# JanEGerken/HEAL-SWIN

Measured on AMD Instinct MI355X. Metric: images/sec fwd+bwd, HEAL-SWIN nside=256 seg, batch=8 at 1/2/4/8 MI355X, higher is better.
Workload: dtype bf16

## Files before the change

### heal_swin_amd/_lib.py

```python
import ctypes
import os

import numpy as np

_PKG = os.path.dirname(os.path.abspath(__file__))
LIB_PATH = os.path.join(_PKG, "lib", "libhealswin.so")

HS_F32, HS_BF16 = 0, 1
HS_F64 = 3
HS_PRED_LABELS, HS_PRED_ROWS16 = 2, 4
HS_ATTN_COSINE = 1
HS_ATTN_FORCE_VALU = 2
HS_ATTN_RESIDUAL = 4
HS_ATTN_OVERWRITE_GRADS = 8
HS_EPI_BIAS, HS_EPI_GELU, HS_EPI_DGELU, HS_EPI_RESID = 0, 1, 2, 3
HS_ACC_DEFER = 2
HS_MLP_NORM_AFTER = 16
HS_U8, HS_I32, HS_I64 = 8, 9, 10
HS_FLAT_PATCH_ROWS, HS_FLAT_PIXEL_ROWS, HS_FLAT_IMAGE = 0, 1, 2
HS_DEPTH_L1, HS_DEPTH_L2, HS_DEPTH_HUBER, HS_DEPTH_LOGVAR = 0, 1, 2, 3
HS_DT_NONE, HS_DT_LOG, HS_DT_INV = 0, 1, 2
HS_DT_ZERO_BKG, HS_DT_1000_BKG, HS_DT_AFFINE, HS_DT_INVERSE = 1, 2, 4, 8
HS_DEPTH_STATS_WORDS = 15

c_i64 = ctypes.c_int64
c_int = ctypes.c_int
c_uint = ctypes.c_uint
c_ptr = ctypes.c_void_p
c_float = ctypes.c_float


class WgradProblem(ctypes.Structure):
    _fields_ = [("dy", c_ptr), ("x", c_ptr), ("dw", c_ptr), ("dbias", c_ptr), ("n_out", c_int), ("k_in", c_int), ("accumulate", c_int),
                ("gelu_x", c_int)]


def wgrad_problems(members):
    arr = (WgradProblem * len(members))()
# ... 339 lines not shown
```

### heal_swin_amd/csrc/gemm_nt.hip

```cpp
#include <cstdlib>

#include "hs_gelu.h"

namespace hs {
HS_DEFINE_SEED_EPOCH_SETTER(set_seed_epoch_gemm_nt)

#ifdef HS_GEMM_TRACE
#define HS_GEMM_TRACE_PARAM uint64_t* trace;
constexpr int kTraceCap = 240;
static uint64_t* g_trace = nullptr;
extern "C" int hs_gemm_nt_set_trace(void* buf) {
    g_trace = (uint64_t*)buf;
    return 0;
}
template <typename Params>
void trace_attach(Params& p) {
    p.trace = g_trace;
}
constexpr int trace_lds(int used, int nw) { return used + nw * kTraceCap * 8 <= 163840 ? nw * kTraceCap * 8 : 0; }
struct Trace {
    uint64_t* out;
    bool on;
    int n = 0, nw, wave, lane;
    uint32_t base;
// ... 21 lines not shown
        }
    }
};
#else
#define HS_GEMM_TRACE_PARAM
template <typename Params>
void trace_attach(Params&) {}
constexpr int trace_lds(int, int) { return 0; }
struct Trace {
    template <typename Params>
    __device__ __forceinline__ Trace(const Params&, bool, uint32_t, int, int, int) {}
    __device__ __forceinline__ void operator()(int) const {}
    __device__ __forceinline__ void flush() const {}
};
#endif

namespace {

typedef unsigned int u32x2 __attribute__((__vector_size__(8)));
typedef unsigned int u32x4v __attribute__((__vector_size__(16)));

constexpr int kStoreAux = 2;
constexpr int kInAux = 2;
enum { EPI_BIAS = 0, EPI_GELU = 1, EPI_DGELU = 2, EPI_RESID = 3 };
constexpr int64_t kMaxRecords = 0x7FFFFE00;

struct GemmParams {
    const uint16_t *a, *b;
    int64_t lda, ldb;
    int k;
    const uint16_t *a2, *b2;
    int64_t lda2, ldb2;
    int k2;
    const float* bias;
    uint16_t* c;
    uint16_t* aux;
    int64_t m;
    int n;
    int tiles_n, tiles, per_xcd, blocks_per_xcd;
    float drop_p;
    uint64_t seed;
    HS_GEMM_TRACE_PARAM
};

template <int BM_, int BN_, int WM_, int WN_, int NSTAGE_, bool ALIAS_, int WGS_PER_CU_>
struct TileTraits {
    static constexpr int BM = BM_, BN = BN_, WM = WM_, WN = WN_, NSTAGE = NSTAGE_, WGS_PER_CU = WGS_PER_CU_;
    static constexpr bool ALIAS = ALIAS_;
    static constexpr int NW = WM * WN;
    static constexpr int TM = BM / WM / 32, TN = BN / WN / 32;
    static constexpr int AB = BM * 128, BB = BN * 128, STAGE = AB + BB;
    static constexpr int AHEAD = NSTAGE - 1;
    static_assert(TN == 2 && (TM == 2 || TM == 4), "the kernel is written for wave tiles of 64 columns and 64 or 128 rows");
    static_assert(!ALIAS || NW * 4096 <= STAGE, "patches do not fit a stage buffer");
    static_assert(BN * 4 <= 1024, "a bias slot holds one 1-KB DMA piece");

    static constexpr bool has_in(int epi) { return epi == EPI_DGELU || epi == EPI_RESID; }
    static constexpr bool ring(int epi) { return has_in(epi) && ALIAS && TM == 4 && STAGE >= NW * 8192; }
    static constexpr bool lbias(int epi) { return ALIAS && epi != EPI_DGELU; }
    static constexpr int NSLOT = NSTAGE + 1;
    static constexpr int PATCH_OFF = NSTAGE * STAGE;
    static constexpr int BIAS_OFF = NSTAGE * STAGE + (ALIAS ? 0 : NW * 4096);
    static constexpr int bias_lds(int epi) { return lbias(epi) ? NSLOT * 1024 : 0; }
    static constexpr int trace_off(int epi) { return BIAS_OFF + bias_lds(epi); }
    static constexpr int lds_bytes(int epi) { return trace_off(epi) + trace_lds(trace_off(epi), NW); }
};
using Tile1 = TileTraits<128, 128, 2, 2, 2, false, 2>;
using Tile2 = TileTraits<256, 128, 4, 2, 3, true, 1>;
using Tile3 = TileTraits<256, 256, 2, 4, 2, true, 1>;

constexpr int epi_younger_ops(int tm, int i) {
    const int stores = i < 2 ? i : 1;
    const int last_d = i + 1 < tm - 1 ? i + 1 : tm - 1;
    return 4 * (stores + (last_d - i));
}

template <int OFF>
__device__ __forceinline__ u32x4 lds_read_b128(uint32_t addr) {
    u32x4 v;
    asm volatile("ds_read_b128 %0, %1 offset:%2" : "=v"(v) : "v"(addr), "n"(OFF));
    return v;
}
// ... 31 lines not shown
        for (int j = 0; j < J; ++j) off[j] = row[j] * ((int)ld * 2) + col[j];
        ld32 = (int)ld * 64;
    }
    __device__ __forceinline__ void issue(unsigned char* stage, int wave, int q, int kb, int kseg) const {
        lds_void* dst = (lds_void*)(stage + LDS + (wave * N + q) * 1024);
        if constexpr (SC) {
            __builtin_amdgcn_raw_ptr_buffer_load_lds(rsrc, dst, 16, (uint32_t)off[q % J], kb + (q >> 2) * ld32, 0, 0);
        } else {
            const uint32_t voff = kb + col[q] < kseg ? (uint32_t)(off[q] + kb) : kOob;
            __builtin_amdgcn_raw_ptr_buffer_load_lds(rsrc, dst, 16, voff, 0, 0, 0);
        }
    }
};
__device__ __forceinline__ uint32_t frag_addr(uint32_t lds_base, int r, int half) {
    const int R = r >> 1;
    return lds_base + R * 256 + (((((r & 1) << 3) + half) ^ (R & 15)) << 4);
}

template <typename Tile, int EPI, bool DROP, bool FAST>
__global__ void __launch_bounds__(Tile::NW * 64, 2) gemm_nt_kernel(GemmParams p) {
#if defined(__HIP_DEVICE_COMPILE__)
    constexpr int BM = Tile::BM, BN = Tile::BN, WM = Tile::WM, WN = Tile::WN, NW = Tile::NW, TM = Tile::TM, TN = Tile::TN;
    constexpr int NSTAGE = Tile::NSTAGE, AHEAD = Tile::AHEAD, NSLOT = Tile::NSLOT, STAGE = Tile::STAGE, BIAS_OFF = Tile::BIAS_OFF;
    constexpr bool ALIAS = Tile::ALIAS, HAS_IN = Tile::has_in(EPI), RING = Tile::ring(EPI), LBIAS = Tile::lbias(EPI);
    constexpr int IW = FAST ? NW / 2 : NW;
    using OperandA = Operand<Tile::AB / 1024 / IW, 0, FAST>;
    using OperandB = Operand<Tile::BB / 1024 / IW, Tile::AB, FAST>;
    constexpr int PIECES = OperandA::N + OperandB::N;
    static_assert(Tile::lds_bytes(EPI) <= 163840, "LDS of one workgroup exceeds 160 KB");
    __shared__ __attribute__((aligned(16))) unsigned char smem[Tile::lds_bytes(EPI)];

    const int tid = threadIdx.x, lane = tid & 63, half = lane >> 5, l31 = lane & 31;
    const int wave = __builtin_amdgcn_readfirstlane(tid >> 6);
    const int wm = wave / WN, wn = wave % WN;

    const int xcd = blockIdx.x & 7, lb = blockIdx.x >> 3;
    const int id_end = min((xcd + 1) * p.per_xcd, p.tiles);
    const int id0 = xcd * p.per_xcd + lb;
    if (id0 >= id_end) return;
    const int nk1 = (p.k + 63) >> 6, nk2 = (p.k2 + 63) >> 6, nk = nk1 + nk2;
    struct Origin {
        int64_t m0;
        int n0;
    };
    auto tile_origin = [&](int id) {
        const int tm = id / p.tiles_n, tn = id - tm * p.tiles_n;
// ... 88 lines not shown
            constexpr int rest = PIECES - ks * PQ, cnt = rest < 0 ? 0 : rest < PQ ? rest : PQ;
            wait_frags(ks_c, Int<(ks < 3 ? TM + TN : 0)>{});
            mma(ks_c, Int<ks * PQ>{}, Int<cnt>{});
            if constexpr (ks + 2 < 4) read_frags(Int<ks + 2>{});
        });
    };

    const uint32_t own_rel = wave * 4096 + l31 * 128 + 8 * half;
    const uint32_t own_out_rel = wave * 4096 + l31 * 128 + 8 * (half ^ ((l31 >> 3) & 1));
    const uint32_t row_rel = wave * 4096 + (lane >> 3) * 128 + (((lane & 7) ^ (lane >> 3)) << 4);
    const bool second_half = ((half ^ (lane & (p.n >> 2))) & 1) != 0;
    auto epilogue = [&](int id, int buf_done, int slot_c) {
        const uint32_t patch_off = ALIAS ? buf_done * STAGE : Tile::PATCH_OFF;
        TR(10);
        if (ALIAS) __builtin_amdgcn_s_barrier();
        TR(11);
        const Origin o = tile_origin(id);
        const int64_t m0 = o.m0;
        const int n2 = p.n * 2;
        const int64_t cbytes = (p.m - m0) * (int64_t)n2;
        const __amdgpu_buffer_rsrc_t rc = clamped_rsrc(p.c + m0 * p.n, p.c ? cbytes : 0);
        const __amdgpu_buffer_rsrc_t rx = clamped_rsrc(p.aux + m0 * p.n, p.aux ? cbytes : 0);
        const ElemRng rng(p.drop_p, p.seed);
        const bool wide = RING || (p.n & 7) == 0;
        const int ncol0 = o.n0 + wn * (BN / WN);
        auto col_of = [&](int j, int g) { return ncol0 + j * 32 + 4 * half + 8 * g; };
        float4 bias4[TN][4];
        const uint32_t baddr = lds0 + BIAS_OFF + slot_c * 1024 + (wn * (BN / WN) + 4 * half) * 4;
        auto lds_bias = [&](int j, float4 (&b)[4]) {
            u32x4 bq[4];
#pragma unroll
            for (int g = 0; g < 4; ++g) asm volatile("ds_read_b128 %0, %1" : "=v"(bq[g]) : "v"(baddr + (j * 32 + 8 * g) * 4));
            asm volatile("s_waitcnt lgkmcnt(0)" : "+v"(bq[0]), "+v"(bq[1]), "+v"(bq[2]), "+v"(bq[3]));
#pragma unroll
            for (int g = 0; g < 4; ++g) b[g] = __builtin_bit_cast(float4, bq[g]);
        };
        if constexpr (!LBIAS) {
#pragma unroll
            for (int j = 0; j < TN; ++j)
#pragma unroll
                for (int g = 0; g < 4; ++g) {
                    const int n = col_of(j, g);
                    bias4[j][g] = (EPI != EPI_DGELU && p.bias && n < p.n) ? *(const float4*)(p.bias + n) : make_float4(0.f, 0.f, 0.f, 0.f);
                }
        }
        const int rl_col = ncol0 + (lane & 7) * 8;
        const uint32_t rl_voff = rl_col < p.n ? (uint32_t)((lane >> 3) * n2 + rl_col * 2) : kOob;
        auto row_soff = [&](int i, int t) -> int { return (wm * (BM / WM) + i * 32 + 8 * t) * n2; };
        const int in_col = ncol0 + (((lane & 7) ^ (lane >> 3)) << 3);
        const uint32_t in_voff = in_col < p.n ? (uint32_t)((lane >> 3) * n2 + in_col * 2) : kOob;
        auto request_in = [&](int i) {
            unsigned char* base = smem + patch_off + (i & 1) * (NW * 4096) + wave * 4096;
#pragma unroll
            for (int t = 0; t < 4; ++t)
                __builtin_amdgcn_raw_ptr_buffer_load_lds(rx, (lds_void*)(base + t * 1024), 16, in_voff, row_soff(i, t), 0, kInAux);
        };
        if constexpr (RING) {
            request_in(0);
            request_in(1);
        }
#pragma unroll
        for (int i = 0; i < TM; ++i) {
            const int ml = wm * (BM / WM) + i * 32 + l31;
            auto direct_off = [&](int j, int g) { return col_of(j, g) < p.n ? (uint32_t)(ml * n2 + col_of(j, g) * 2) : kOob; };
            const uint32_t pbase = lds0 + patch_off + (RING ? (i & 1) * (NW * 4096) : 0);
            const uint32_t own_addr = pbase + own_rel, row_addr = pbase + row_rel, own_out = pbase + own_out_rel;
// ... 25 lines not shown
                } else {
#pragma unroll
                    for (int j = 0; j < TN; ++j)
#pragma unroll
                        for (int g = 0; g < 4; ++g) xin[j][g] = __builtin_amdgcn_raw_buffer_load_b64(rx, direct_off(j, g), 0, 0);
                }
            }
            auto chunk_key = [&](int j, int g) { return rng.chunk_key((uint64_t)((m0 + ml) * p.n + col_of(j, g)) >> 3); };
            auto keep2 = [&](uint32_t ck, int t) {
                const uint32_t hh = ElemRng::pair_bits(ck, ElemRng::half_mult(second_half, t));
                return f32x2{rng.keep_lo(hh), rng.keep_hi(hh)};
            };
            u32x2 o1[TN][4], o2[TN][4];
#pragma unroll
            for (int j = 0; j < TN; ++j) {
                if constexpr (LBIAS) lds_bias(j, bias4[j]);
#pragma unroll
                for (int g = 0; g < 4; ++g) {
                    f32x16& a16 = acc[j][i];
                    f32x2 v[2] = {f32x2{a16[4 * g], a16[4 * g + 1]} + f32x2{bias4[j][g].x, bias4[j][g].y},
                                  f32x2{a16[4 * g + 2], a16[4 * g + 3]} + f32x2{bias4[j][g].z, bias4[j][g].w}};
                    uint32_t ck = 0;
                    if (DROP) ck = chunk_key(j, g);
                    if (EPI == EPI_GELU) {
                        o1[j][g] = pack_bf16x4(v[0], v[1]);
                        a16[4 * g] = v[0].x; a16[4 * g + 1] = v[0].y; a16[4 * g + 2] = v[1].x; a16[4 * g + 3] = v[1].y;
                        continue;
                    } else {
                        if (EPI == EPI_DGELU || EPI == EPI_RESID) {
#pragma unroll
                            for (int t = 0; t < 2; ++t) {
                                const f32x2 x = {__uint_as_float(xin[j][g][t] << 16), __uint_as_float(xin[j][g][t] & 0xffff0000u)};
                                if (EPI == EPI_DGELU) {
                                    v[t] *= gelu_grad2(x);
                                    if (DROP) v[t] *= keep2(ck, t);
                                } else {
                                    v[t] += x;
                                }
                            }
                        }
                        o1[j][g] = pack_bf16x4(v[0], v[1]);
                    }
#pragma unroll
                    for (int r = 0; r < 4; ++r) a16[4 * g + r] = 0.f;
                }
            }
            auto make_o2 = [&]() {
#pragma unroll
                for (int j = 0; j < TN; ++j)
#pragma unroll
                    for (int g0 = 0; g0 < 4; g0 += 2) {
                        f32x16& a16 = acc[j][i];
                        f32x2 v[4] = {f32x2{a16[4 * g0], a16[4 * g0 + 1]}, f32x2{a16[4 * g0 + 2], a16[4 * g0 + 3]},
                                      f32x2{a16[4 * g0 + 4], a16[4 * g0 + 5]}, f32x2{a16[4 * g0 + 6], a16[4 * g0 + 7]}};
#pragma unroll
                        for (int t = 0; t < 4; ++t) v[t] = gelu2(v[t]);
#pragma unroll
                        for (int gg = 0; gg < 2; ++gg) {
                            const int g = g0 + gg;
                            if (DROP) {
                                const uint32_t ck = chunk_key(j, g);
#pragma unroll
                                for (int t = 0; t < 2; ++t) v[2 * gg + t] *= keep2(ck, t);
                            }
                            o2[j][g] = pack_bf16x4(v[2 * gg], v[2 * gg + 1]);
#pragma unroll
                            for (int r = 0; r < 4; ++r) a16[4 * g + r] = 0.f;
                        }
                    }
            };
            TR(20);
            auto emit = [&](const __amdgpu_buffer_rsrc_t& rs, const u32x2 (&o)[TN][4]) {
                if (wide) {
#pragma unroll
                    for (int j = 0; j < TN; ++j)
#pragma unroll
                        for (int g = 0; g < 4; ++g)
                            asm volatile("ds_write_b64 %0, %1" ::"v"(own_out + (((4 * j + g) ^ (l31 & 7)) << 4)), "v"(o[j][g]) : "memory");
                    u32x4 rws[4];
                    asm volatile("ds_read_b128 %0, %1" : "=v"(rws[0]) : "v"(row_addr));
                    asm volatile("ds_read2_b64 %0, %1 offset0:129 offset1:128" : "=v"(rws[1]) : "v"(row_addr));
                    asm volatile("ds_read_b128 %0, %1 offset:2048" : "=v"(rws[2]) : "v"(row_addr));
                    asm volatile("ds_read2_b64 %0, %1 offset0:129 offset1:128" : "=v"(rws[3]) : "v"(row_addr + 2048));
                    asm volatile("s_waitcnt lgkmcnt(0)" : "+v"(rws[0]), "+v"(rws[1]), "+v"(rws[2]), "+v"(rws[3]));
                    TR(22);
#pragma unroll
                    for (int t = 0; t < 4; ++t)
                        __builtin_amdgcn_raw_buffer_store_b128(__builtin_bit_cast(u32x4v, rws[t]), rs, rl_voff, row_soff(i, t), kStoreAux);
                    asm volatile("s_nop 0" ::"v"(rws[0]), "v"(rws[1]), "v"(rws[2]), "v"(rws[3]));
                } else {
#pragma unroll
                    for (int j = 0; j < TN; ++j)
#pragma unroll
                        for (int g = 0; g < 4; ++g) __builtin_amdgcn_raw_buffer_store_b64(o[j][g], rs, direct_off(j, g), 0, kStoreAux);
                }
            };
            if (EPI == EPI_GELU) {
                if (NW == 8 && wave >= NW / 2) {
                    make_o2();
                    emit(rx, o2);
                    TR(21);
                    __builtin_amdgcn_sched_barrier(0);
                    if (p.c) emit(rc, o1);
                } else {
                    if (p.c) emit(rc, o1);
                    TR(21);
                    __builtin_amdgcn_sched_barrier(0);
                    make_o2();
                    emit(rx, o2);
                }
            } else {
                emit(rc, o1);
            }
            if constexpr (RING) {
                if (i + 2 < TM) request_in(i + 2);
            }
            TR(12 + i);
        }
    };

// ... 5 lines not shown
        ++ks_i;
        if (ks_i == nk) {
            ks_i = 0;
            id_i += stride;
            if (id_i < id_end) retarget(id_i, nk1 == 0, true);
        } else if (ks_i == nk1) {
            retarget(id_i, true, false);
        }
    };
    auto kb_of = [&](int ks) { return (ks >= nk1 ? ks - nk1 : ks) * 128; };
    retarget(id_i, false, true);
    int issued = 0;
#pragma unroll
    for (int q = 0; q < AHEAD; ++q) {
        if (id_i < id_end) {
            issue_pieces(kb_of(ks_i), q, Int<0>{}, Int<PIECES>{});
            advance_issue();
            ++issued;
        }
    }
    int buf = 0, buf_free = AHEAD;
    bool drained = false;
    constexpr int LATER = (AHEAD - 1) * PIECES;
    constexpr int kEpiOps = TM * 4;
    TR(0);
    while (true) {
        TR(3);
        if (IW < NW && wave >= IW) {
        } else if (AHEAD > 1 && issued == AHEAD && !drained)
            wait_pieces_behind<LATER, 0>();
        else if (drained && issued == AHEAD)
            wait_pieces_behind<LATER, kEpiOps>();
        else if (drained && issued == 1)
            wait_pieces_behind<0, kEpiOps>();
        else
            wait_pieces_behind<0, 0>();
        drained = false;
        TR(1);
        __builtin_amdgcn_s_barrier();
        TR(2);
        const bool more = id_i < id_end;
        const bool last = ks_c + 1 == nk;
        compute(buf, more, kb_of(ks_i), buf_free);
        --issued;
        if (more) {
            advance_issue();
            ++issued;
// ... 8 lines not shown
            ks_c = 0;
            id_c += stride;
            if (id_c >= id_end) break;
        } else {
            ++ks_c;
        }
    }
    TR.flush();
#endif
}

template <typename Tile, bool FAST>
int launch_tile(GemmParams& p, int epi, hipStream_t s) {
    const int tiles_m = (int)((p.m + Tile::BM - 1) / Tile::BM);
    p.tiles_n = (p.n + Tile::BN - 1) / Tile::BN;
    const int64_t tiles = (int64_t)tiles_m * p.tiles_n;
    if (tiles > 0x7fffffff) return fail(HS_ERR_UNSUPPORTED, "too many output tiles");
    p.tiles = (int)tiles;
    p.per_xcd = (p.tiles + 7) / 8;
    const int resident = usable_cus_per_xcd() * Tile::WGS_PER_CU;
    p.blocks_per_xcd = p.per_xcd < resident ? p.per_xcd : resident;
    const dim3 grid((unsigned)(8 * p.blocks_per_xcd)), block(Tile::NW * 64);
    using Kernel = void (*)(GemmParams);
    static constexpr Kernel kKernels[4][2] = {
        {gemm_nt_kernel<Tile, EPI_BIAS, false, FAST>, gemm_nt_kernel<Tile, EPI_BIAS, false, FAST>},
        {gemm_nt_kernel<Tile, EPI_GELU, false, FAST>, gemm_nt_kernel<Tile, EPI_GELU, true, FAST>},
        {gemm_nt_kernel<Tile, EPI_DGELU, false, FAST>, gemm_nt_kernel<Tile, EPI_DGELU, true, FAST>},
        {gemm_nt_kernel<Tile, EPI_RESID, false, FAST>, gemm_nt_kernel<Tile, EPI_RESID, false, FAST>}};
    hipLaunchKernelGGL(kKernels[epi][p.drop_p > 0.f], grid, block, 0, s, p);
    HS_LAUNCH_CHECK("gemm_nt");
    return HS_OK;
}

}

int gemm_nt_check_shape(const char* who, int64_t lda, int64_t ldb, int k, int64_t lda2, int64_t ldb2, int k2, int64_t m, int n) {
    HS_CHECK_ARG(m > 0 && n > 0 && k > 0 && k2 >= 0, "%s: empty shape", who);
    if (k % 8 || k2 % 8 || lda % 8 || ldb % 8 || (k2 && (lda2 % 8 || ldb2 % 8)) || n % 4)
        return fail(HS_ERR_UNSUPPORTED, "%s: k, k2 and the row strides must be multiples of 8, n a multiple of 4", who);
    if (lda * 2 * 256 > kMaxRecords || ldb * 2 * 256 > kMaxRecords || (int64_t)n * 2 * 256 > kMaxRecords)
        return fail(HS_ERR_UNSUPPORTED, "%s: row stride too large", who);
    if (((m + 127) / 128) * (((int64_t)n + 127) / 128) > 0x7fffffff) return fail(HS_ERR_UNSUPPORTED, "%s: too many output tiles", who);
    return HS_OK;
}

int gemm_nt_tile_variant(int forced, int64_t m, int n, int k, int k2, int epilogue) {
    int variant = forced;
    if (!variant) {
        const int64_t tiles2 = ((m + 255) / 256) * ((n + 127) / 128), tiles3 = ((m + 255) / 256) * ((n + 255) / 256);
        if (tiles2 < 256)
            variant = 1;
        else if ((epilogue == EPI_GELU || epilogue == EPI_DGELU) ? n >= 512 : (n >= 1024 && k + k2 >= 512))
            variant = 3;
        else if (n >= 256 && tiles3 >= 768 && k % 64 == 0 && k2 % 64 == 0)
            variant = 3;
        else
            variant = 2;
    }
    if (variant == 3 && (epilogue == EPI_DGELU || epilogue == EPI_RESID) && n % 8) variant = 2;
    return variant == 2 || variant == 3 ? variant : 1;
}

}

namespace {
int g_tile_variant = 0;
}

extern "C" {

int hs_gemm_nt_set_tile(int variant) {
    g_tile_variant = variant;
    return HS_OK;
}

int hs_gemm_nt_tile_variant(int64_t m, int n, int k, int k2, int epilogue) {
    return hs::gemm_nt_tile_variant(g_tile_variant, m, n, k, k2, epilogue);
}

int hs_gemm_nt(const void* a, int64_t lda, const void* b, int64_t ldb, int k, const void* a2, int64_t lda2, const void* b2,
               int64_t ldb2, int k2, const float* bias, void* c, void* aux, int64_t m, int n, int epilogue, float drop_p,
               uint64_t seed, int dtype, void* stream) {
    using namespace hs;
    HS_CHECK_ARG(dtype == HS_BF16, "hs_gemm_nt: bf16 activations only (fp32 runs use the library GEMM)");
    HS_CHECK_ARG(a && b && m > 0 && n > 0 && k > 0, "hs_gemm_nt: null operand or empty shape");
    HS_CHECK_ARG(epilogue >= EPI_BIAS && epilogue <= EPI_RESID, "hs_gemm_nt: unknown epilogue %d", epilogue);
    HS_CHECK_ARG(k2 == 0 || (a2 && b2 && k2 > 0), "hs_gemm_nt: second segment needs a2, b2, k2 > 0");
    HS_CHECK_ARG(c || (epilogue == EPI_GELU && aux), "hs_gemm_nt: no output");
    HS_CHECK_ARG(epilogue == EPI_BIAS || aux, "hs_gemm_nt: this epilogue needs aux");
    HS_CHECK_ARG(drop_p >= 0.f && drop_p <= 1.f, "hs_gemm_nt: drop_p must be in [0, 1]");
    HS_CHECK_ALIGNED("hs_gemm_nt", 16, a, b, a2, b2, bias, c, aux);
    if (int st = gemm_nt_check_shape("hs_gemm_nt", lda, ldb, k, lda2, ldb2, k2, m, n)) return st;
    GemmParams p{};
    p.a = (const uint16_t*)a; p.b = (const uint16_t*)b; p.lda = lda; p.ldb = ldb; p.k = k;
    p.a2 = (const uint16_t*)a2; p.b2 = (const uint16_t*)b2; p.lda2 = lda2; p.ldb2 = ldb2; p.k2 = k2;
    p.bias = bias; p.c = (uint16_t*)c; p.aux = (uint16_t*)aux; p.m = m; p.n = n;
    p.drop_p = drop_p; p.seed = seed;
    trace_attach(p);
    hipStream_t st = (hipStream_t)stream;
    const bool fast = k % 64 == 0 && k2 % 64 == 0;
    switch (gemm_nt_tile_variant(g_tile_variant, m, n, k, k2, epilogue)) {
        case 2: return fast ? launch_tile<Tile2, true>(p, epilogue, st) : launch_tile<Tile2, false>(p, epilogue, st);
        case 3: return fast ? launch_tile<Tile3, true>(p, epilogue, st) : launch_tile<Tile3, false>(p, epilogue, st);
        default: return launch_tile<Tile1, false>(p, epilogue, st);
    }
}

}
```

### heal_swin_amd/csrc/hs_gelu.h

```cpp
#pragma once
#include "hs_device.h"

namespace hs {

constexpr float kGeluP0 = -1.000002567e+00f, kGeluP1 = -1.151043788e+00f, kGeluP2 = -4.594249196e-01f, kGeluP3 = -5.234669296e-02f,
                kGeluP4 = 7.289804275e-03f, kGeluP5 = -5.021511049e-04f;
constexpr float kGeluE2 = -0.7213475204444817f;
constexpr float kGeluE0 = -1.3257480647361595f;

__device__ __forceinline__ float gelu_tail(float a) {
    float p = fmaf(kGeluP5, a, kGeluP4);
    p = fmaf(p, a, kGeluP3);
    p = fmaf(p, a, kGeluP2);
    p = fmaf(p, a, kGeluP1);
    p = fmaf(p, a, kGeluP0);
    return __builtin_amdgcn_exp2f(p);
}
__device__ __forceinline__ float gelu_f(float x) {
    const float a = fabsf(x);
    return fmaf(-a, gelu_tail(a), fmaxf(x, 0.f));
}
__device__ __forceinline__ float gelu_grad_f(float x) {
    const float h = gelu_tail(fabsf(x));
    const float e = __builtin_amdgcn_exp2f(fmaf(x * x, kGeluE2, kGeluE0));
// ... 2 lines not shown

typedef float f32x2 __attribute__((ext_vector_type(2)));
__device__ __forceinline__ f32x2 gelu_tail2(f32x2 a) {
    f32x2 p = a * kGeluP5 + kGeluP4;
    p = p * a + kGeluP3;
    p = p * a + kGeluP2;
    p = p * a + kGeluP1;
    p = p * a + kGeluP0;
    return f32x2{__builtin_amdgcn_exp2f(p.x), __builtin_amdgcn_exp2f(p.y)};
}
__device__ __forceinline__ f32x2 gelu2(f32x2 x) {
    const f32x2 a = {fabsf(x.x), fabsf(x.y)};
    const f32x2 relu = {fmaxf(x.x, 0.f), fmaxf(x.y, 0.f)};
    return relu - a * gelu_tail2(a);
}
__device__ __forceinline__ f32x2 gelu_grad2(f32x2 x) {
    const f32x2 a = {fabsf(x.x), fabsf(x.y)};
    const f32x2 w = 0.5f - gelu_tail2(a);
    const f32x2 s = (x * x) * kGeluE2 + kGeluE0;
    const f32x2 e = {__builtin_amdgcn_exp2f(s.x), __builtin_amdgcn_exp2f(s.y)};
    const f32x2 cdf = f32x2{copysignf(w.x, x.x), copysignf(w.y, x.y)} + 0.5f;
    return x * e + cdf;
}

}
```

### heal_swin_amd/ops/gemm.py

```python
import math
import os

import torch

from .. import _lib
from .._lib import check, lib, ptr, stream_ptr
from . import runtime
from .runtime import RT, _aligned, _cast_param, _defer_flag, _defer_keep, _require_gpu, _sink_buffer, _timed


OWN_GEMM = os.environ.get("HS_OWN_GEMM", "auto")


OWN_GELU_MAX_K = 4096
OWN_DGELU_MAX_K = 1024
OWN_BIAS_MAX_K = 0


class GemmTuner:
    MIN_FLOP = 1 << 33

    def __init__(self):
        self.picks = {}
        self.trials = {}
# ... 31 lines not shown
                        gemm_nt(a, w, bias32)
                    else:
                        torch.nn.functional.linear(a, w, bias16)
                    e1.record()
                    e1.synchronize()
                    if rep:
                        best[own] = min(best[own], e0.elapsed_time(e1))
            del sets
        self.trials[key] = (round(1e3 * best[True], 1), round(1e3 * best[False], 1))
        self.picks[key] = best[True] <= best[False]
        return self.picks[key]


GEMM_TUNE = True
GEMM_TUNER = GemmTuner()


def own_gemm_ok(epi, n, k, dtype, k2=0, m=None):
    if dtype != torch.bfloat16 or OWN_GEMM == "0" or k % 8 or k2 % 8 or n % 8 or n < 16:
        return False
    if OWN_GEMM == "1" or RT.prefer_own_gemm:
        return True
    kk = k + k2
    if epi == _lib.HS_EPI_DGELU:
        return kk <= OWN_DGELU_MAX_K
    if epi == _lib.HS_EPI_GELU:
        return kk <= OWN_GELU_MAX_K
    if OWN_BIAS_MAX_K > 0:
        return kk <= OWN_BIAS_MAX_K
    if GEMM_TUNE and m is not None and k2 == 0 and torch.cuda.is_available():
        pick = GEMM_TUNER.pick(int(m), n, kk, torch.device("cuda", torch.cuda.current_device()))
        if pick is not None:
            return pick
    return kk <= 128 or n <= 128 or (n <= 256 and kk <= 256)


RESID_DGRAD_OWN = True


def own_gemm_legal(n, k, dtype):
    return dtype == torch.bfloat16 and OWN_GEMM != "0" and k % 8 == 0 and n % 8 == 0 and n >= 16


RESID_EPILOGUE = True


def gemm_nt(a2d, w, bias=None, epi=0, aux=None, a2=None, w2=None, want_c=True, drop_p=0.0, seed=0):
    w, w2, bias = _aligned(w), _aligned(w2), _aligned(bias)
    if epi != _lib.HS_EPI_GELU:
        aux = _aligned(aux)
    m, k = a2d.shape
    n = w.shape[0]
    assert a2d.stride(1) == 1 and w.stride(1) == 1 and a2d.dtype == torch.bfloat16 and w.dtype == torch.bfloat16
    c = torch.empty((m, n), dtype=torch.bfloat16, device=a2d.device) if want_c else None
    if epi == _lib.HS_EPI_GELU:
        aux = torch.empty((m, n), dtype=torch.bfloat16, device=a2d.device)
    k2 = 0 if a2 is None else a2.shape[1]
    if bias is not None and bias.dtype != torch.float32:
        bias = bias.float()
    with _timed(f"hs_gemm_nt epi={epi} m={m} n={n} k={k + k2}", a2d.device, 2 * (m * (k + k2) + n * (k + k2) + m * n * (2 if (epi and want_c) else 1)), 2 * m * n * (k + k2)):
        check(lib.hs_gemm_nt(ptr(a2d), a2d.stride(0), ptr(w), w.stride(0), k, ptr(a2), 0 if a2 is None else a2.stride(0), ptr(w2),
                             0 if w2 is None else w2.stride(0), k2, ptr(bias), ptr(c), ptr(aux), m, n, epi, float(drop_p), int(seed),
                             _lib.HS_BF16, stream_ptr(a2d.device)), "hs_gemm_nt")
    return c, aux


def _lib_tag(kind, m, n, k):
    return f"lib {kind} m={m} n={n} k={k}"


FP32_GEMM = os.environ.get("HS_FP32_GEMM", "bf16x3")
_BF16X3_MIN = 160
_SPLIT_MEMO = []
_MM_OUT_DTYPE = [None]


def _bf16x3_ok(x, n=None, k=None):
    ok = FP32_GEMM == "bf16x3" and x.dtype == torch.float32 and x.is_cuda and x.shape[-1] % 8 == 0
# ... 361 lines not shown
```

### heal_swin_amd/ops/mlp_branch.py

```python
import os

import torch

from .. import _lib
from .._lib import check, lib, ptr, stream_ptr
from .runtime import RT, _aligned, _cast_param, _defer_flag, _defer_keep, _draw_seed, _extras, _f32, _require_gpu, _timed
from .norm import _norm_param_grads, _norm_param_result
from .gemm import (_Split, _bf16x3_ok, _cast_param_t, _input_grad, _lib_linear, _lib_matmul, _param_grads, _split_of, gemm_nt, own_gemm_legal, own_gemm_ok)


class MlpFn(torch.autograd.Function):

    @staticmethod
    def forward(ctx, x, w1, b1, w2, b2, drop_p, seed, passthrough, residual=None):
        _require_gpu(x, w1, b1, w2, b2, residual)
        c_in, hid = w1.shape[1], w1.shape[0]
        x2 = x.reshape(-1, c_in)
        if not x2.is_contiguous():
            x2 = x2.contiguous()
        dt = x.dtype
        x3 = a3 = None
        w1c, w2c = _cast_param(w1, dt), _cast_param(w2, dt)
        need_grad = any(ctx.needs_input_grad[:5])
        if own_gemm_ok(_lib.HS_EPI_GELU, hid, c_in, dt):
            h, a = gemm_nt(x2, w1c, b1, _lib.HS_EPI_GELU, want_c=need_grad, drop_p=drop_p, seed=seed)
        else:
            h = _lib_linear(x2, w1c, None if b1 is None else _cast_param(b1, dt))
            x3 = _split_of(x2)
            if _bf16x3_ok(h, w2.shape[0], hid) and w2c.dtype == torch.float32 and w2.shape[0] % 8 == 0 and hid % 8 == 0:
                h = _aligned(h)
                a3 = torch.empty((h.shape[0], 3 * hid), dtype=torch.bfloat16, device=h.device)
                check(lib.hs_gelu_split3(None, ptr(h), ptr(a3), h.shape[0], hid, float(drop_p), int(seed), stream_ptr(h.device)),
                      "hs_gelu_split3")
                a = _Split(a3, hid)
            else:
                a = torch.empty_like(h)
                check(lib.hs_gelu_fwd(ptr(h), ptr(a), h.numel(), float(drop_p), int(seed), _lib.dtype_code(dt), stream_ptr(h.device)),
                      "hs_gelu_fwd")
        ctx.has_residual = residual is not None
        if residual is not None and own_gemm_legal(w2.shape[0], hid, dt):
            res2 = residual.reshape(-1, w2.shape[0])
            y = gemm_nt(a, w2c, b2, _lib.HS_EPI_RESID, aux=res2 if res2.is_contiguous() else res2.contiguous())[0]
        elif own_gemm_ok(_lib.HS_EPI_BIAS, w2.shape[0], hid, dt):
            y = gemm_nt(a, w2c, b2)[0]
        else:
            y = _lib_linear(a, w2c, None if b2 is None else _cast_param(b2, dt))
            a3 = _split_of(a)
# ... 4 lines not shown
        assert not isinstance(a, _Split)
        ctx.save_for_backward(None if x3 is not None else x2, h, None if a3 is not None else a, w1, w2)
        ctx.biases = (b1, b2)
        ctx.casts = (w1c if w1c.dtype != w1.dtype else None, w2c if w2c.dtype != w2.dtype else None)
        ctx.cast_cache = RT.cast_cache
        ctx.meta = (float(drop_p), int(seed), x.shape)
        ctx.splits = (x3, a3)
        y = y.view(x.shape[:-1] + (w2.shape[0],))
        return (y, x.view_as(x)) if passthrough else y

    @staticmethod
    def backward(ctx, dy, dx_res=None):
        x2, h, a, w1, w2 = ctx.saved_tensors
        b1, b2 = ctx.biases
        w1c, w2c = ctx.casts
        p, seed, xshape = ctx.meta
        if dy is None:
            return dx_res, None, None, None, None, None, None, None, None
        c_out, hid, c_in = w2.shape[0], w1.shape[0], w1.shape[1]
        dy2 = dy.reshape(-1, c_out)
        if not dy2.is_contiguous():
            dy2 = dy2.contiguous()
        dt = dy2.dtype
        if own_gemm_ok(_lib.HS_EPI_DGELU, hid, c_out, dt):
            dh = gemm_nt(dy2, _cast_param_t(w2, dt, ctx.cast_cache), None, _lib.HS_EPI_DGELU, aux=h, drop_p=p, seed=seed)[0]
        else:
            da = _lib_matmul(dy2, w2c if (w2c is not None and w2c.dtype == dt) else w2.to(dt))
            if _bf16x3_ok(da, c_in, hid) and w1.dtype == torch.float32 and c_in % 8 == 0 and hid % 8 == 0:
                dh3 = torch.empty((h.shape[0], 3 * hid), dtype=torch.bfloat16, device=h.device)
                check(lib.hs_gelu_split3(ptr(_aligned(da)), ptr(_aligned(h)), ptr(dh3), h.shape[0], hid, p, seed, stream_ptr(h.device)), "hs_gelu_split3")
                dh = _Split(dh3, hid)
            else:
                dh = torch.empty_like(h)
                check(lib.hs_gelu_bwd(ptr(da), ptr(h), ptr(dh), h.numel(), p, seed, _lib.dtype_code(dt), stream_ptr(h.device)), "hs_gelu_bwd")
            del da
        dx = None
        if ctx.needs_input_grad[0]:
            dx = _input_grad(dh, w1, w1c, None if dx_res is None else dx_res.reshape(-1, c_in), ctx.cast_cache).reshape(xshape)
        ctx.casts = ctx.cast_cache = None
        (x3, a3), ctx.splits = ctx.splits, (None, None)
        dw2, db2 = _param_grads(dy2, a, w2, b2, ctx.needs_input_grad[3], b2 is not None and ctx.needs_input_grad[4], a3)
        dw1, db1 = _param_grads(dh, x2, w1, b1, ctx.needs_input_grad[1], b1 is not None and ctx.needs_input_grad[2], x3)
        return dx, dw1, db1, dw2, db2, None, None, None, (dy if ctx.has_residual else None)


def mlp(x, w1, b1, w2, b2, drop_p=0.0, seed=None, passthrough=False, residual=None):
    if drop_p > 0.0 and seed is None:
        seed = _draw_seed()
    return MlpFn.apply(x, w1, b1, w2, b2, float(drop_p), int(seed or 0), bool(passthrough), residual)


FUSED_MLP = os.environ.get("HS_FUSED_MLP", "1") != "0"
MLP_KEEP_ACT = True


def fused_mlp_ok(x, hidden):
    c = x.shape[-1]
    return bool(FUSED_MLP and x.is_cuda and x.dtype == torch.bfloat16 and (x.numel() // c) % 32 == 0 and
                lib.hs_mlp_fused_supported(int(c), int(hidden), _lib.HS_BF16))


class FusedMlpBlockFn(torch.autograd.Function):

    @staticmethod
    def forward(ctx, x, ln_w, ln_b, w1, b1, w2, b2, post_norm=False, stoch=None):
        _require_gpu(x, ln_w, ln_b, w1, b1, w2, b2)
        assert stoch is None or post_norm
        C, hid = x.shape[-1], w1.shape[0]
        x2 = x.reshape(-1, C)
        if not x2.is_contiguous():
            x2 = x2.contiguous()
        rows = x2.shape[0]
        dev = x.device
        need = any(ctx.needs_input_grad)
        w1c, w2c = _cast_param(w1, torch.bfloat16).contiguous(), _cast_param(w2, torch.bfloat16).contiguous()
        g, b = _f32(ln_w), _f32(ln_b)
# ... 94 lines not shown
```

### include/healswin.h

```cpp
#ifndef HEALSWIN_H
#define HEALSWIN_H

#include <stdint.h>

#ifdef __cplusplus
extern "C" {
#endif

typedef enum {
    HS_OK = 0,
    HS_ERR_INVALID_ARG = 1,
    HS_ERR_UNSUPPORTED = 2,
    HS_ERR_HIP = 3,
    HS_ERR_NOT_PERMUTATION = 4,
    HS_ERR_MISALIGNED = 5
} hs_status;

typedef enum { HS_F32 = 0, HS_BF16 = 1 } hs_dtype;

#define HS_ATTN_COSINE 1u
#define HS_ATTN_FORCE_VALU 2u
#define HS_ATTN_RESIDUAL 4u
#define HS_ATTN_OVERWRITE_GRADS 8u

// ... 205 lines not shown
                              int64_t n_tokens, int channels, int num_heads, int window_size, unsigned flags, int dtype,
                              void* stream);

int hs_window_attn_module_fwd_train(const void* x, void* out, void* xn_out, float* mean_out, float* rstd_out, void* qkv_out,
                                    void* attn_out, float* lse_out, const void* qkv_w, const float* qkv_b, const void* proj_w,
                                    const float* proj_b, const float* ln_gamma, const float* ln_beta, const float* bias,
                                    const float* head_scale, const int32_t* idx, int64_t roll, const uint8_t* labels,
                                    const float* norm2_gamma, const float* norm2_beta, void* n2_out, float* mean2_out, float* rstd2_out,
                                    int batch, int64_t n_tokens, int channels, int num_heads, int window_size, unsigned flags, int dtype,
                                    void* stream);

int64_t hs_window_attn_module_bwd_chain_workspace(int batch, int64_t n_tokens, int channels, int num_heads, int window_size);
int hs_window_attn_module_bwd_chain(const void* dout, const void* x, const void* xn, const float* mean, const float* rstd, const void* qkv,
                              const void* attn_out, const float* lse, const void* qkv_w_t, const void* proj_w_t, const float* ln_gamma,
                              const float* bias, const float* head_scale, const int32_t* idx, int64_t roll, const uint8_t* labels,
                              void* dx, float* dqkv_w, float* dqkv_b, float* dproj_w, float* dproj_b, float* dln_gamma, float* dln_beta,
                              float* dbias, float* dhead_scale, float* workspace, int accumulate, int batch, int64_t n_tokens, int channels,
                              int num_heads, int window_size, unsigned flags, int dtype, void* stream);

#define HS_EPI_BIAS 0
#define HS_EPI_GELU 1
#define HS_EPI_DGELU 2
#define HS_EPI_RESID 3
int hs_gemm_nt(const void* a, int64_t lda, const void* b, int64_t ldb, int k, const void* a2, int64_t lda2, const void* b2,
               int64_t ldb2, int k2, const float* bias, void* c, void* aux, int64_t m, int n, int epilogue, float drop_p,
               uint64_t seed, int dtype, void* stream);
int hs_gemm_nt_set_tile(int variant);
int hs_gemm_nt_tile_variant(int64_t m, int n, int k, int k2, int epilogue);

int hs_pix2ang_nest(int nside, int64_t first, int64_t count, double* theta, double* phi);
int hs_sample_bilinear_u8(const void* img, int batch, int channels, int height, int width, const double* rx, const double* ry,
                          int64_t n, void* out, void* stream);
int hs_sample_mask_u8(const void* mask, int batch, int height, int width, const double* rx, const double* ry, int64_t n,
                      int background, void* out, void* stream);

#define HS_PRED_LABELS 2
#define HS_PRED_ROWS16 4
int hs_hp_interp_weights_nest(int nside, const double* theta, const double* phi, int64_t n, int64_t* pix, double* wgt);
int hs_backproject_labels(const void* pred, int pred_kind, int64_t batch, int64_t npix, int n_classes, int64_t stride_b,
                          int64_t stride_k, int64_t stride_p, const int32_t* nearest, int64_t n_out, int background, uint8_t* out,
                          void* stream);
int hs_backproject_image(const uint8_t* hp_img, int64_t planes, int64_t npix, const int32_t* idx, const double* wgt, int64_t n_out,
                         double* out, void* stream);
int hs_seg_confusion(const void* pred, int pred_kind, int64_t batch, int64_t npix, int n_classes, int64_t stride_b, int64_t stride_k,
                     int64_t stride_p, const int32_t* nearest, int64_t n_out, const uint8_t* target, int uncovered, int64_t* conf,
                     int64_t* bad, void* stream);
// ... 148 lines not shown
```

Before: 57.11.

## Store GELU derivative in fc1 epilogue and multiply it in fc2 backward

Adds a GELU_G epilogue that computes the GELU activation and its derivative together in the fc1 GEMM, writing the derivative in place of the pre-activation. A new DMUL epilogue in the fc2 data-gradient GEMM then multiplies by the stored derivative instead of recomputing gelu_grad from the pre-activation. The MLP branch uses this path by default when dropout is off and the activation is kept. This moves the transcendental derivative work from backward into forward and changes the epilogue scheduling, with the derivative now rounded to bf16.

```diff
diff --git a/heal_swin_amd/_lib.py b/heal_swin_amd/_lib.py
--- a/heal_swin_amd/_lib.py
+++ b/heal_swin_amd/_lib.py
@@ -13,7 +13,7 @@
 HS_ATTN_FORCE_VALU = 2
 HS_ATTN_RESIDUAL = 4
 HS_ATTN_OVERWRITE_GRADS = 8
-HS_EPI_BIAS, HS_EPI_GELU, HS_EPI_DGELU, HS_EPI_RESID = 0, 1, 2, 3
+HS_EPI_BIAS, HS_EPI_GELU, HS_EPI_DGELU, HS_EPI_RESID, HS_EPI_GELU_G, HS_EPI_DMUL = 0, 1, 2, 3, 4, 5
 HS_ACC_DEFER = 2
 HS_MLP_NORM_AFTER = 16
 HS_U8, HS_I32, HS_I64 = 8, 9, 10
diff --git a/heal_swin_amd/csrc/gemm_nt.hip b/heal_swin_amd/csrc/gemm_nt.hip
--- a/heal_swin_amd/csrc/gemm_nt.hip
+++ b/heal_swin_amd/csrc/gemm_nt.hip
@@ -67,7 +67,11 @@
 
 constexpr int kStoreAux = 2;
 constexpr int kInAux = 2;
-enum { EPI_BIAS = 0, EPI_GELU = 1, EPI_DGELU = 2, EPI_RESID = 3 };
+enum { EPI_BIAS = 0, EPI_GELU = 1, EPI_DGELU = 2, EPI_RESID = 3, EPI_GELU_G = 4, EPI_DMUL = 5, EPI_COUNT = 6 };
+constexpr bool epi_has_in(int epi) { return epi == EPI_DGELU || epi == EPI_RESID || epi == EPI_DMUL; }
+constexpr bool epi_has_bias(int epi) { return epi != EPI_DGELU && epi != EPI_DMUL; }
+constexpr bool epi_gelu_class(int epi) { return epi == EPI_GELU || epi == EPI_DGELU || epi == EPI_GELU_G || epi == EPI_DMUL; }
+constexpr int epi_min_ops(int epi, int tm) { return (epi == EPI_GELU_G ? 2 : 1) * 4 * tm; }
 constexpr int64_t kMaxRecords = 0x7FFFFE00;
 
 struct GemmParams {
@@ -100,9 +104,9 @@
     static_assert(!ALIAS || NW * 4096 <= STAGE, "patches do not fit a stage buffer");
     static_assert(BN * 4 <= 1024, "a bias slot holds one 1-KB DMA piece");
 
-    static constexpr bool has_in(int epi) { return epi == EPI_DGELU || epi == EPI_RESID; }
+    static constexpr bool has_in(int epi) { return epi_has_in(epi); }
     static constexpr bool ring(int epi) { return has_in(epi) && ALIAS && TM == 4 && STAGE >= NW * 8192; }
-    static constexpr bool lbias(int epi) { return ALIAS && epi != EPI_DGELU; }
+    static constexpr bool lbias(int epi) { return ALIAS && epi_has_bias(epi); }
     static constexpr int NSLOT = NSTAGE + 1;
     static constexpr int PATCH_OFF = NSTAGE * STAGE;
     static constexpr int BIAS_OFF = NSTAGE * STAGE + (ALIAS ? 0 : NW * 4096);
@@ -180,6 +184,8 @@
 #if defined(__HIP_DEVICE_COMPILE__)
     constexpr int BM = Tile::BM, BN = Tile::BN, WM = Tile::WM, WN = Tile::WN, NW = Tile::NW, TM = Tile::TM, TN = Tile::TN;
     constexpr int NSTAGE = Tile::NSTAGE, AHEAD = Tile::AHEAD, NSLOT = Tile::NSLOT, STAGE = Tile::STAGE, BIAS_OFF = Tile::BIAS_OFF;
+    constexpr bool TWO_PATCH = EPI == EPI_GELU_G && Tile::ALIAS && Tile::STAGE >= NW * 8192;
+    constexpr uint32_t kPatch2 = NW * 4096;
     constexpr bool ALIAS = Tile::ALIAS, HAS_IN = Tile::has_in(EPI), RING = Tile::ring(EPI), LBIAS = Tile::lbias(EPI);
     constexpr int IW = FAST ? NW / 2 : NW;
     using OperandA = Operand<Tile::AB / 1024 / IW, 0, FAST>;
@@ -314,7 +320,7 @@
         const __amdgpu_buffer_rsrc_t rc = clamped_rsrc(p.c + m0 * p.n, p.c ? cbytes : 0);
         const __amdgpu_buffer_rsrc_t rx = clamped_rsrc(p.aux + m0 * p.n, p.aux ? cbytes : 0);
         const ElemRng rng(p.drop_p, p.seed);
-        const bool wide = RING || (p.n & 7) == 0;
+        const bool wide = RING || EPI == EPI_GELU_G || (p.n & 7) == 0;
         const int ncol0 = o.n0 + wn * (BN / WN);
         auto col_of = [&](int j, int g) { return ncol0 + j * 32 + 4 * half + 8 * g; };
         float4 bias4[TN][4];
@@ -333,7 +339,7 @@
 #pragma unroll
                 for (int g = 0; g < 4; ++g) {
                     const int n = col_of(j, g);
-                    bias4[j][g] = (EPI != EPI_DGELU && p.bias && n < p.n) ? *(const float4*)(p.bias + n) : make_float4(0.f, 0.f, 0.f, 0.f);
+                    bias4[j][g] = (epi_has_bias(EPI) && p.bias && n < p.n) ? *(const float4*)(p.bias + n) : make_float4(0.f, 0.f, 0.f, 0.f);
                 }
         }
         const int rl_col = ncol0 + (lane & 7) * 8;
@@ -405,18 +411,23 @@
                                   f32x2{a16[4 * g + 2], a16[4 * g + 3]} + f32x2{bias4[j][g].z, bias4[j][g].w}};
                     uint32_t ck = 0;
                     if (DROP) ck = chunk_key(j, g);
-                    if (EPI == EPI_GELU) {
+                    if (EPI == EPI_GELU_G) {
+                        a16[4 * g] = v[0].x; a16[4 * g + 1] = v[0].y; a16[4 * g + 2] = v[1].x; a16[4 * g + 3] = v[1].y;
+                        continue;
+                    } else if (EPI == EPI_GELU) {
                         o1[j][g] = pack_bf16x4(v[0], v[1]);
                         a16[4 * g] = v[0].x; a16[4 * g + 1] = v[0].y; a16[4 * g + 2] = v[1].x; a16[4 * g + 3] = v[1].y;
                         continue;
                     } else {
-                        if (EPI == EPI_DGELU || EPI == EPI_RESID) {
+                        if (HAS_IN) {
 #pragma unroll
                             for (int t = 0; t < 2; ++t) {
                                 const f32x2 x = {__uint_as_float(xin[j][g][t] << 16), __uint_as_float(xin[j][g][t] & 0xffff0000u)};
                                 if (EPI == EPI_DGELU) {
                                     v[t] *= gelu_grad2(x);
                                     if (DROP) v[t] *= keep2(ck, t);
+                                } else if (EPI == EPI_DMUL) {
+                                    v[t] = f32x2{a16[4 * g + 2 * t], a16[4 * g + 2 * t + 1]} * x;
                                 } else {
                                     v[t] += x;
                                 }
@@ -453,13 +464,15 @@
                     }
             };
             TR(20);
-            auto emit = [&](const __amdgpu_buffer_rsrc_t& rs, const u32x2 (&o)[TN][4]) {
-                if (wide) {
-#pragma unroll
-                    for (int j = 0; j < TN; ++j)
-#pragma unroll
-                        for (int g = 0; g < 4; ++g)
-                            asm volatile("ds_write_b64 %0, %1" ::"v"(own_out + (((4 * j + g) ^ (l31 & 7)) << 4)), "v"(o[j][g]) : "memory");
+            auto put = [&](auto wide_c, const __amdgpu_buffer_rsrc_t& rs, int j, int g, u32x2 o, uint32_t poff) {
+                if constexpr (decltype(wide_c)::value)
+                    asm volatile("ds_write_b64 %0, %1" ::"v"(own_out + poff + (((4 * j + g) ^ (l31 & 7)) << 4)), "v"(o) : "memory");
+                else
+                    __builtin_amdgcn_raw_buffer_store_b64(o, rs, direct_off(j, g), 0, kStoreAux);
+            };
+            auto store_rows = [&](const __amdgpu_buffer_rsrc_t& rs, uint32_t poff) {
+                {
+                    const uint32_t row_addr = pbase + row_rel + poff;
                     u32x4 rws[4];
                     asm volatile("ds_read_b128 %0, %1" : "=v"(rws[0]) : "v"(row_addr));
                     asm volatile("ds_read2_b64 %0, %1 offset0:129 offset1:128" : "=v"(rws[1]) : "v"(row_addr));
@@ -471,14 +484,45 @@
                     for (int t = 0; t < 4; ++t)
                         __builtin_amdgcn_raw_buffer_store_b128(__builtin_bit_cast(u32x4v, rws[t]), rs, rl_voff, row_soff(i, t), kStoreAux);
                     asm volatile("s_nop 0" ::"v"(rws[0]), "v"(rws[1]), "v"(rws[2]), "v"(rws[3]));
-                } else {
-#pragma unroll
-                    for (int j = 0; j < TN; ++j)
-#pragma unroll
-                        for (int g = 0; g < 4; ++g) __builtin_amdgcn_raw_buffer_store_b64(o[j][g], rs, direct_off(j, g), 0, kStoreAux);
                 }
             };
-            if (EPI == EPI_GELU) {
+            auto emit = [&](const __amdgpu_buffer_rsrc_t& rs, const u32x2 (&o)[TN][4]) {
+                if (wide) {
+#pragma unroll
+                    for (int j = 0; j < TN; ++j)
+#pragma unroll
+                        for (int g = 0; g < 4; ++g) put(Int<1>{}, rs, j, g, o[j][g], 0);
+                    store_rows(rs, 0);
+                } else {
+#pragma unroll
+                    for (int j = 0; j < TN; ++j)
+#pragma unroll
+                        for (int g = 0; g < 4; ++g) put(Int<0>{}, rs, j, g, o[j][g], 0);
+                }
+            };
+            auto make_o12 = [&]() {
+#pragma unroll
+                for (int j = 0; j < TN; ++j)
+#pragma unroll
+                    for (int g = 0; g < 4; ++g) {
+                        f32x16& a16 = acc[j][i];
+                        f32x2 act[2], der[2];
+#pragma unroll
+                        for (int t = 0; t < 2; ++t) gelu_and_grad2(f32x2{a16[4 * g + 2 * t], a16[4 * g + 2 * t + 1]}, act[t], der[t]);
+                        put(Int<1>{}, rx, j, g, pack_bf16x4(act[0], act[1]), 0);
+                        if constexpr (TWO_PATCH) put(Int<1>{}, rc, j, g, pack_bf16x4(der[0], der[1]), kPatch2);
+                        else o1[j][g] = pack_bf16x4(der[0], der[1]);
+#pragma unroll
+                        for (int r = 0; r < 4; ++r) a16[4 * g + r] = 0.f;
+                    }
+                store_rows(rx, 0);
+                TR(21);
+                if constexpr (TWO_PATCH) store_rows(rc, kPatch2);
+                else emit(rc, o1);
+            };
+            if (EPI == EPI_GELU_G) {
+                make_o12();
+            } else if (EPI == EPI_GELU) {
                 if (NW == 8 && wave >= NW / 2) {
                     make_o2();
                     emit(rx, o2);
@@ -530,7 +574,7 @@
     int buf = 0, buf_free = AHEAD;
     bool drained = false;
     constexpr int LATER = (AHEAD - 1) * PIECES;
-    constexpr int kEpiOps = TM * 4;
+    constexpr int kEpiOps = epi_min_ops(EPI, TM);
     TR(0);
     while (true) {
         TR(3);
@@ -585,11 +629,13 @@
     p.blocks_per_xcd = p.per_xcd < resident ? p.per_xcd : resident;
     const dim3 grid((unsigned)(8 * p.blocks_per_xcd)), block(Tile::NW * 64);
     using Kernel = void (*)(GemmParams);
-    static constexpr Kernel kKernels[4][2] = {
+    static constexpr Kernel kKernels[EPI_COUNT][2] = {
         {gemm_nt_kernel<Tile, EPI_BIAS, false, FAST>, gemm_nt_kernel<Tile, EPI_BIAS, false, FAST>},
         {gemm_nt_kernel<Tile, EPI_GELU, false, FAST>, gemm_nt_kernel<Tile, EPI_GELU, true, FAST>},
         {gemm_nt_kernel<Tile, EPI_DGELU, false, FAST>, gemm_nt_kernel<Tile, EPI_DGELU, true, FAST>},
-        {gemm_nt_kernel<Tile, EPI_RESID, false, FAST>, gemm_nt_kernel<Tile, EPI_RESID, false, FAST>}};
+        {gemm_nt_kernel<Tile, EPI_RESID, false, FAST>, gemm_nt_kernel<Tile, EPI_RESID, false, FAST>},
+        {gemm_nt_kernel<Tile, EPI_GELU_G, false, FAST>, nullptr},
+        {gemm_nt_kernel<Tile, EPI_DMUL, false, FAST>, nullptr}};
     hipLaunchKernelGGL(kKernels[epi][p.drop_p > 0.f], grid, block, 0, s, p);
     HS_LAUNCH_CHECK("gemm_nt");
     return HS_OK;
@@ -613,14 +659,14 @@
         const int64_t tiles2 = ((m + 255) / 256) * ((n + 127) / 128), tiles3 = ((m + 255) / 256) * ((n + 255) / 256);
         if (tiles2 < 256)
             variant = 1;
-        else if ((epilogue == EPI_GELU || epilogue == EPI_DGELU) ? n >= 512 : (n >= 1024 && k + k2 >= 512))
+        else if (epi_gelu_class(epilogue) ? n >= 512 : (n >= 1024 && k + k2 >= 512))
             variant = 3;
         else if (n >= 256 && tiles3 >= 768 && k % 64 == 0 && k2 % 64 == 0)
             variant = 3;
         else
             variant = 2;
     }
-    if (variant == 3 && (epilogue == EPI_DGELU || epilogue == EPI_RESID) && n % 8) variant = 2;
+    if (variant == 3 && epi_has_in(epilogue) && n % 8) variant = 2;
     return variant == 2 || variant == 3 ? variant : 1;
 }
 
@@ -647,9 +693,12 @@
     using namespace hs;
     HS_CHECK_ARG(dtype == HS_BF16, "hs_gemm_nt: bf16 activations only (fp32 runs use the library GEMM)");
     HS_CHECK_ARG(a && b && m > 0 && n > 0 && k > 0, "hs_gemm_nt: null operand or empty shape");
-    HS_CHECK_ARG(epilogue >= EPI_BIAS && epilogue <= EPI_RESID, "hs_gemm_nt: unknown epilogue %d", epilogue);
+    HS_CHECK_ARG(epilogue >= EPI_BIAS && epilogue < EPI_COUNT, "hs_gemm_nt: unknown epilogue %d", epilogue);
     HS_CHECK_ARG(k2 == 0 || (a2 && b2 && k2 > 0), "hs_gemm_nt: second segment needs a2, b2, k2 > 0");
     HS_CHECK_ARG(c || (epilogue == EPI_GELU && aux), "hs_gemm_nt: no output");
+    if (epilogue == EPI_GELU_G && n % 8) return fail(HS_ERR_UNSUPPORTED, "hs_gemm_nt: HS_EPI_GELU_G needs n to be a multiple of 8");
+    HS_CHECK_ARG((epilogue != EPI_GELU_G && epilogue != EPI_DMUL) || drop_p == 0.f,
+                 "hs_gemm_nt: HS_EPI_GELU_G / HS_EPI_DMUL are deterministic (dropout runs HS_EPI_GELU / HS_EPI_DGELU)");
     HS_CHECK_ARG(epilogue == EPI_BIAS || aux, "hs_gemm_nt: this epilogue needs aux");
     HS_CHECK_ARG(drop_p >= 0.f && drop_p <= 1.f, "hs_gemm_nt: drop_p must be in [0, 1]");
     HS_CHECK_ALIGNED("hs_gemm_nt", 16, a, b, a2, b2, bias, c, aux);
diff --git a/heal_swin_amd/csrc/hs_gelu.h b/heal_swin_amd/csrc/hs_gelu.h
--- a/heal_swin_amd/csrc/hs_gelu.h
+++ b/heal_swin_amd/csrc/hs_gelu.h
@@ -48,5 +48,16 @@
     const f32x2 cdf = f32x2{copysignf(w.x, x.x), copysignf(w.y, x.y)} + 0.5f;
     return x * e + cdf;
 }
+__device__ __forceinline__ void gelu_and_grad2(f32x2 x, f32x2& act, f32x2& grad) {
+    const f32x2 a = {fabsf(x.x), fabsf(x.y)};
+    const f32x2 relu = {fmaxf(x.x, 0.f), fmaxf(x.y, 0.f)};
+    const f32x2 h = gelu_tail2(a);
+    act = relu - a * h;
+    const f32x2 w = 0.5f - h;
+    const f32x2 s = (x * x) * kGeluE2 + kGeluE0;
+    const f32x2 e = {__builtin_amdgcn_exp2f(s.x), __builtin_amdgcn_exp2f(s.y)};
+    const f32x2 cdf = f32x2{copysignf(w.x, x.x), copysignf(w.y, x.y)} + 0.5f;
+    grad = x * e + cdf;
+}
 
 }
diff --git a/heal_swin_amd/ops/gemm.py b/heal_swin_amd/ops/gemm.py
--- a/heal_swin_amd/ops/gemm.py
+++ b/heal_swin_amd/ops/gemm.py
@@ -77,9 +77,9 @@
     if OWN_GEMM == "1" or RT.prefer_own_gemm:
         return True
     kk = k + k2
-    if epi == _lib.HS_EPI_DGELU:
+    if epi in (_lib.HS_EPI_DGELU, _lib.HS_EPI_DMUL):
         return kk <= OWN_DGELU_MAX_K
-    if epi == _lib.HS_EPI_GELU:
+    if epi in (_lib.HS_EPI_GELU, _lib.HS_EPI_GELU_G):
         return kk <= OWN_GELU_MAX_K
     if OWN_BIAS_MAX_K > 0:
         return kk <= OWN_BIAS_MAX_K
@@ -102,13 +102,14 @@
 
 def gemm_nt(a2d, w, bias=None, epi=0, aux=None, a2=None, w2=None, want_c=True, drop_p=0.0, seed=0):
     w, w2, bias = _aligned(w), _aligned(w2), _aligned(bias)
-    if epi != _lib.HS_EPI_GELU:
+    two_out = epi in (_lib.HS_EPI_GELU, _lib.HS_EPI_GELU_G)
+    if not two_out:
         aux = _aligned(aux)
     m, k = a2d.shape
     n = w.shape[0]
     assert a2d.stride(1) == 1 and w.stride(1) == 1 and a2d.dtype == torch.bfloat16 and w.dtype == torch.bfloat16
     c = torch.empty((m, n), dtype=torch.bfloat16, device=a2d.device) if want_c else None
-    if epi == _lib.HS_EPI_GELU:
+    if two_out:
         aux = torch.empty((m, n), dtype=torch.bfloat16, device=a2d.device)
     k2 = 0 if a2 is None else a2.shape[1]
     if bias is not None and bias.dtype != torch.float32:
diff --git a/heal_swin_amd/ops/mlp_branch.py b/heal_swin_amd/ops/mlp_branch.py
--- a/heal_swin_amd/ops/mlp_branch.py
+++ b/heal_swin_amd/ops/mlp_branch.py
@@ -22,7 +22,11 @@
         x3 = a3 = None
         w1c, w2c = _cast_param(w1, dt), _cast_param(w2, dt)
         need_grad = any(ctx.needs_input_grad[:5])
-        if own_gemm_ok(_lib.HS_EPI_GELU, hid, c_in, dt):
+        ctx.stored_grad = bool(GELU_STORE_GRAD and MLP_KEEP_ACT and need_grad and drop_p == 0.0 and
+                               own_gemm_ok(_lib.HS_EPI_GELU_G, hid, c_in, dt) and own_gemm_ok(_lib.HS_EPI_DMUL, hid, w2.shape[0], dt))
+        if ctx.stored_grad:
+            h, a = gemm_nt(x2, w1c, b1, _lib.HS_EPI_GELU_G)
+        elif own_gemm_ok(_lib.HS_EPI_GELU, hid, c_in, dt):
             h, a = gemm_nt(x2, w1c, b1, _lib.HS_EPI_GELU, want_c=need_grad, drop_p=drop_p, seed=seed)
         else:
             h = _lib_linear(x2, w1c, None if b1 is None else _cast_param(b1, dt))
@@ -73,7 +77,9 @@
         if not dy2.is_contiguous():
             dy2 = dy2.contiguous()
         dt = dy2.dtype
-        if own_gemm_ok(_lib.HS_EPI_DGELU, hid, c_out, dt):
+        if ctx.stored_grad:
+            dh = gemm_nt(dy2, _cast_param_t(w2, dt, ctx.cast_cache), None, _lib.HS_EPI_DMUL, aux=h)[0]
+        elif own_gemm_ok(_lib.HS_EPI_DGELU, hid, c_out, dt):
             dh = gemm_nt(dy2, _cast_param_t(w2, dt, ctx.cast_cache), None, _lib.HS_EPI_DGELU, aux=h, drop_p=p, seed=seed)[0]
         else:
             da = _lib_matmul(dy2, w2c if (w2c is not None and w2c.dtype == dt) else w2.to(dt))
@@ -103,6 +109,7 @@
 
 FUSED_MLP = os.environ.get("HS_FUSED_MLP", "1") != "0"
 MLP_KEEP_ACT = True
+GELU_STORE_GRAD = os.environ.get("HS_GELU_STORE_GRAD", "1") != "0"
 
 
 def fused_mlp_ok(x, hidden):
diff --git a/include/healswin.h b/include/healswin.h
--- a/include/healswin.h
+++ b/include/healswin.h
@@ -251,6 +251,8 @@
 #define HS_EPI_GELU 1
 #define HS_EPI_DGELU 2
 #define HS_EPI_RESID 3
+#define HS_EPI_GELU_G 4
+#define HS_EPI_DMUL 5
 int hs_gemm_nt(const void* a, int64_t lda, const void* b, int64_t ldb, int k, const void* a2, int64_t lda2, const void* b2,
                int64_t ldb2, int k2, const float* bias, void* c, void* aux, int64_t m, int n, int epilogue, float drop_p,
                uint64_t seed, int dtype, void* stream);
```

Result: no change. 57.64, median of 6 (+0.9%).
